# kabachuha/sd-webui-text2video

Measured on NVIDIA H100. Metric: denoised frames/sec (UNet+VAE) ModelScope 24fx256^2 50-step, higher is better.
Workload: dtype f16 (fp32 accumulate / norms / softmax)

## Files before the change

sd-webui-text2video_b200/csrc/api.cu:

```cuda
#include "../../include/t2v_b200.h"
#include "common.cuh"
#include "gemm_tc.cuh"
#include "kernels.cuh"

#include <cstdarg>
#include <cstdlib>
#include <cstdio>
#include <cstring>

namespace t2v {

static char g_err[512] = "";
static int g_device = -1;
static int g_num_sms = 132;
static void* g_gn_ws = nullptr;
static size_t g_gn_ws_bytes = 0;

void set_error(const char* fmt, ...) {
    va_list ap;
    va_start(ap, fmt);
    vsnprintf(g_err, sizeof(g_err), fmt, ap);
    va_end(ap);
}
int num_sms() { return g_num_sms; }
// ... 55 lines not shown
}
const char* t2v_last_error(void) { return g_err; }
int t2v_num_sms(void) { return g_num_sms; }
const char* t2v_version(void) { return "t2v_b200 0.2 (sm_90a; wgmma+TMA implicit GEMM)"; }

int t2v_op_gemm(const void* a, long long lda, int K, int nd, const int* dims, int ntaps, const int* tap_off,
                const void* w_packed, int n_alloc, int N, int b_batch_dim, int flags, void* out, long long ldo,
                const void* bias, int bias_rows, long long bias_stride, const void* residual, long long ldr,
                float alpha, int force_bn, int force_cg, void* stream) {
    GemmProblem p;
    memset(&p, 0, sizeof(p));
    p.a = reinterpret_cast<const __half*>(a);
    p.lda = lda;
    p.K = K;
    p.nd = nd;
    for (int d = 0; d < nd; ++d) p.dim[d] = dims[d];
    p.ntaps = ntaps;
    for (int t = 0; t < ntaps; ++t)
        for (int d = 0; d < nd; ++d) p.tap_off[t][d] = tap_off ? tap_off[t * nd + d] : 0;
    p.b = reinterpret_cast<const __half*>(w_packed);
    p.n_alloc = n_alloc;
    p.N = N;
    p.b_batch_dim = b_batch_dim;
    p.flags = flags & ~(GEMM_DBG_FORCE_BS | GEMM_DBG_NO_BS);
    p.force_bs = (flags & GEMM_DBG_FORCE_BS) ? 1 : ((flags & GEMM_DBG_NO_BS) ? -1 : 0);
    p.out = out;
    p.ldo = ldo;
    p.bias = reinterpret_cast<const __half*>(bias);
    p.bias_rows = bias_rows;
    p.bias_stride = bias_stride;
    p.residual = reinterpret_cast<const __half*>(residual);
    p.ldr = ldr;
    p.alpha = alpha;
    p.force_bn = force_bn;
    p.force_cg = force_cg;
    GemmPlan plan;
    int rc = gemm_plan(p, &plan, g_num_sms);
    if (rc != 0) {
        set_error("gemm_plan failed (%d)", rc);
        return rc;
    }
    rc = gemm_launch(plan, reinterpret_cast<cudaStream_t>(stream));
    if (rc != 0) set_error("gemm_launch failed: %s", cudaGetErrorString(cudaGetLastError()));
    return rc;
}

int t2v_latent_blend(const float* image_latents, int image_frames, const double* noise, const double* weights, double* out,
                     double* mask_out, int BC, int F, long long hw, void* stream) {
// ... 116 lines not shown
```

sd-webui-text2video_b200/csrc/gemm_tc.cu:

```cuda
#include "common.cuh"
#include "gemm_tc.cuh"
#include "ptx.cuh"

#include <algorithm>
#include <cstdio>
#include <cstdlib>
#include <cstring>

namespace t2v {

namespace {

constexpr int kThreads = 384;
constexpr int kRegsProducer = 40;
constexpr int kRegsConsumer = 232;
constexpr int kABytes = GEMM_BLOCK_M * GEMM_BLOCK_K * 2;
constexpr int kSmemBudget = 216 * 1024;
constexpr int kMaxStages = 8;
constexpr int kEpiRowBytes = 128;
constexpr int kEpiWarpBytes = 8 * kEpiRowBytes + 16 * 4;
constexpr int kEpiBytes = 8 * kEpiWarpBytes;

template <int BN>
struct Cfg {
    static constexpr int kBBytes = BN * GEMM_BLOCK_K * 2;
    static constexpr int kStageBytes = kABytes + kBBytes;
    static constexpr int kStages = (kSmemBudget / kStageBytes) > kMaxStages ? kMaxStages : (kSmemBudget / kStageBytes);
    static constexpr int kColBytes = BN * 8;
    static constexpr int kTailBytes = 1024  + 256  + kEpiBytes + kColBytes;
    static constexpr int kSmemBytes = kStages * kStageBytes + kTailBytes;
    static constexpr int kBsSmemBytes = kSmemBudget + kTailBytes;
    static_assert(kSmemBytes <= 227 * 1024, "shared memory per block");
};

__device__ __forceinline__ float gelu_erf(float x) {
    const float z = fabsf(x) * 0.70710678118654752440f;
    float t;
    asm("rcp.approx.ftz.f32 %0, %1;" : "=f"(t) : "f"(fmaf(0.3275911f, z, 1.0f)));
    float p = fmaf(t, 0.5f * 1.061405429f, 0.5f * -1.453152027f);
    p = fmaf(p, t, 0.5f * 1.421413741f);
    p = fmaf(p, t, 0.5f * -0.284496736f);
    p = fmaf(p, t, 0.5f * 0.254829592f);
    const float q = p * t * ex2_approx(z * z * -1.4426950408889634f);
    return x * (x < 0.f ? q : 1.0f - q);
}

__device__ __forceinline__ uint32_t stg_off(int r, int b, int segs) {
    const int L = r * segs + (b >> 4);
    return static_cast<uint32_t>(((L ^ ((L >> 3) & 7)) << 4) | (b & 15));
}

template <int BN, bool GEGLU>
__device__ __forceinline__ void epilogue_affine(const GemmDesc& g, float (&acc)[BN / 2], const uint8_t* cols, const int* rowg,
                                                const float2 (&rs)[2], int tn, int lane) {
    const int quad = lane & 3, fr = lane >> 2;
    if (g.bias != nullptr && g.bias_rows > 0 && (g.flags & GEMM_LN) == 0) {
        const int nvalid = GEGLU ? g.N / 2 : g.N;
        const __half* brow[2];
#pragma unroll
        for (int h = 0; h < 2; ++h) {
            const int fg = rowg[fr + 8 * h];
            brow[h] = g.bias + (fg >= 0 ? (fg / g.bias_rows) * g.bias_stride : 0);
        }
#pragma unroll
        for (int j = 0; j < BN / 8; ++j) {
#pragma unroll
            for (int e = 0; e < 2; ++e) {
                const int col = tn * BN + 8 * j + 2 * quad + e;
                if (!GEGLU && col >= nvalid) continue;
                acc[4 * j + e] = fmaf(acc[4 * j + e], g.alpha, __half2float(__ldg(brow[0] + col)));
                acc[4 * j + 2 + e] = fmaf(acc[4 * j + 2 + e], g.alpha, __half2float(__ldg(brow[1] + col)));
            }
        }
        return;
    }
    const bool ln = (g.flags & GEMM_LN) != 0;
#pragma unroll
    for (int j = 0; j < BN / 8; ++j) {
        const int c = 8 * j + 2 * quad;
        if (ln) {
            const float4 p = *reinterpret_cast<const float4*>(cols + 8 * c);
            acc[4 * j] = fmaf(rs[0].y, fmaf(-rs[0].x, p.x, acc[4 * j]), p.y);
            acc[4 * j + 2] = fmaf(rs[1].y, fmaf(-rs[1].x, p.x, acc[4 * j + 2]), p.y);
            acc[4 * j + 1] = fmaf(rs[0].y, fmaf(-rs[0].x, p.z, acc[4 * j + 1]), p.w);
            acc[4 * j + 3] = fmaf(rs[1].y, fmaf(-rs[1].x, p.z, acc[4 * j + 3]), p.w);
        } else {
            const float2 b = __half22float2(*reinterpret_cast<const __half2*>(cols + 2 * c));
            acc[4 * j] = fmaf(acc[4 * j], g.alpha, b.x);
            acc[4 * j + 2] = fmaf(acc[4 * j + 2], g.alpha, b.x);
            acc[4 * j + 1] = fmaf(acc[4 * j + 1], g.alpha, b.y);
            acc[4 * j + 3] = fmaf(acc[4 * j + 3], g.alpha, b.y);
        }
    }
}
// ... 91 lines not shown
            const int idx = lane + 32 * p;
            if (idx >= 8 * segs) continue;
            const int gr = rowg[8 * h + idx / segs];
            if (gr < 0) continue;
            const int col = ocol0 + c * CW + EPS * (idx % segs);
            const uint4 val = *reinterpret_cast<const uint4*>(stg + stg_off(idx / segs, 16 * (idx % segs), segs));
            uint8_t* dst = static_cast<uint8_t*>(g.out) + ((F32 ? sp * g.split_stride : 0) + gr * g.ldo + col) * ES;
            if (vec_out && col + EPS <= nvalid) {
                *reinterpret_cast<uint4*>(dst) = val;
            } else {
                const uint32_t w[4] = {val.x, val.y, val.z, val.w};
#pragma unroll
                for (int e = 0; e < EPS; ++e)
                    if (col + e < nvalid) {
                        if constexpr (F32) reinterpret_cast<uint32_t*>(dst)[e] = w[e];
                        else reinterpret_cast<uint16_t*>(dst)[e] = static_cast<uint16_t>(w[e >> 1] >> (16 * (e & 1)));
                    }
            }
        }
        __syncwarp();
    }
}

template <int BN, bool GEGLU, int CG, bool BS = false>
__global__ void __launch_bounds__(kThreads, 1) gemm_tc_kernel(const __grid_constant__ GemmDesc g) {
    using Cf = Cfg<BN>;
    static_assert(!BS || CG == 1, "B-stationary tiles are single-CTA");
    static_assert(!BS || Cf::kBsSmemBytes <= 227 * 1024, "shared memory per block");
    constexpr int kBarStages = BS ? kMaxStages : Cf::kStages;
    const uint32_t rank = CG == 2 ? cluster_ctarank() : 0u;
    extern __shared__ uint8_t smem_raw[];
    const uint32_t raw = smem_u32(smem_raw);
    uint8_t* smem = smem_raw + (((raw + 1023u) & ~1023u) - raw);
    uint64_t* bars = reinterpret_cast<uint64_t*>(smem + (BS ? kSmemBudget : Cf::kStages * Cf::kStageBytes));
    uint64_t* full = bars;
    uint64_t* empty = bars + kBarStages;
    uint64_t* bfull = empty + kBarStages;
    uint64_t* colfull = bfull + 1;
    uint64_t* colempty = bfull + 2;
    uint8_t* const epi = reinterpret_cast<uint8_t*>(bars) + 256;
    uint8_t* const cols = epi + kEpiBytes;
    const int nst = BS ? g.bs_stages : Cf::kStages;
    uint8_t* const sB_res = smem;
    uint8_t* const sA_ring = smem + (BS ? g.ntaps * g.k_chunks * Cf::kBBytes : 0);

    const int wg = threadIdx.x >> 7;

    if (threadIdx.x == 0) {
        tma_prefetch_desc(&g.map_a);
        tma_prefetch_desc(&g.map_b);
        for (int i = 0; i < kBarStages; ++i) {
            mbar_init(&full[i], 1);
            mbar_init(&empty[i], 2 * CG);
        }
        if constexpr (BS) mbar_init(bfull, 1);
        mbar_init(colfull, 1);
        mbar_init(colempty, 8);
        fence_barrier_init();
    }
    if constexpr (CG == 2) cluster_sync_all();
    else __syncthreads();
    griddep_wait();

    const int pairs_m = (g.tiles_m + CG - 1) / CG;
    const int nsplit = g.splits > 1 ? g.splits : 1;
    const int total_pairs = pairs_m * g.tiles_n * nsplit;
    const int k_total = g.ntaps * g.k_chunks;
    const int k_per = g.splits > 1 ? g.k_per_split : k_total;
    const int bs_tn = BS ? static_cast<int>(blockIdx.x) % g.tiles_n : 0;
    const int first_pair = BS ? static_cast<int>(blockIdx.x) / g.tiles_n : static_cast<int>(blockIdx.x) / CG;
    const int pair_stride = BS ? (static_cast<int>(gridDim.x) - bs_tn + g.tiles_n - 1) / g.tiles_n : static_cast<int>(gridDim.x) / CG;
    const int total_items = BS ? g.tiles_m : total_pairs;
    const bool col_operands = (g.flags & GEMM_LN) != 0 || g.bias == nullptr || g.bias_rows == 0;

    if (wg == 0) {
        setmaxnreg_dec<kRegsProducer>();
        if (threadIdx.x < 32 && elect_one()) {
            int stage = 0;
            uint32_t phase = 0;
            if constexpr (BS) {
// ... 4 lines not shown
                        tma_load_3d(sB_res + it * Cf::kBBytes, &g.map_b, bfull, kc * GEMM_BLOCK_K, bs_tn * BN, tap);
                        if (++kc == kch0) {
                            kc = 0;
                            ++tap;
                        }
                    }
                }
            }
            const int kch = g.k_chunks, nd = g.nd, a_tx = g.a_tx_bytes, tiles_n_ = g.tiles_n, tiles_m_ = g.tiles_m;
            const int bdim = g.b_batch_dim;
            for (int wi = first_pair; wi < total_items; wi += pair_stride) {
                int sp = 0, pt = wi;
                if (!BS && nsplit > 1) {
                    sp = wi % nsplit;
                    pt = wi / nsplit;
                }
                const int it0 = sp * k_per, it1 = min(k_total, it0 + k_per);
                int tn = bs_tn, tmi = wi;
                if constexpr (!BS) {
                    const int pm = pt / tiles_n_;
                    tn = pt - pm * tiles_n_;
                    tmi = pm * CG + static_cast<int>(rank);
                }
                int org[GEMM_MAX_RDIMS] = {0, 0, 0, 0};
                if (nd == 1) {
                    org[0] = tmi * g.box[0];
                } else {
                    int tm = tmi;
#pragma unroll
                    for (int d = 0; d < GEMM_MAX_RDIMS; ++d) {
                        if (d < nd) {
                            const int td = g.tdim[d];
                            const int qd = tm / td;
                            org[d] = (tm - qd * td) * g.box[d];
                            tm = qd;
                        }
                    }
                }
                if (tmi >= tiles_m_) org[0] = g.dim[0];
                const int bbatch = bdim < 0 ? 0 : (bdim == 0 ? org[0] : (bdim == 1 ? org[1] : (bdim == 2 ? org[2] : org[3])));
                int tap = 0, kc = it0;
                if (it0 >= kch) {
                    tap = it0 / kch;
                    kc = it0 - tap * kch;
                }
                int c1 = org[0] + g.tap_off[tap][0], c2 = org[1] + g.tap_off[tap][1];
                int c3 = org[2] + g.tap_off[tap][2], c4 = org[3] + g.tap_off[tap][3];
                for (int it = it0; it < it1; ++it) {
                    mbar_wait(&empty[stage], phase ^ 1u);
                    uint8_t* sa = BS ? sA_ring + stage * kABytes : smem + stage * Cf::kStageBytes;
                    uint8_t* sb = sa + kABytes;
                    const int k0 = kc * GEMM_BLOCK_K;
                    mbar_expect_tx(&full[stage], static_cast<uint32_t>(a_tx + (BS ? 0 : Cf::kBBytes)));
                    if (nd == 1) tma_load_2d(sa, &g.map_a, &full[stage], k0, c1);
                    else if (nd == 2) tma_load_3d(sa, &g.map_a, &full[stage], k0, c1, c2);
                    else if (nd == 3) tma_load_4d(sa, &g.map_a, &full[stage], k0, c1, c2, c3);
                    else tma_load_5d(sa, &g.map_a, &full[stage], k0, c1, c2, c3, c4);
                    if constexpr (CG == 2) {
                        constexpr int kHalf = BN / 2;
                        tma_load_3d_mc(sb + rank * (kHalf * GEMM_BLOCK_K * 2), &g.map_b, &full[stage], k0,
                                       tn * BN + static_cast<int>(rank) * kHalf, tap + bbatch, static_cast<uint16_t>(3));
// ... 18 lines not shown
            }
            griddep_launch();
        } else if (threadIdx.x >= 32 && threadIdx.x < 64 && col_operands) {
            const int lane = threadIdx.x & 31;
            const bool ln = (g.flags & GEMM_LN) != 0;
            uint32_t cphase = 0;
            for (int wi = first_pair; wi < total_items; wi += pair_stride) {
                const int col0 = (BS ? bs_tn : (wi / nsplit) % g.tiles_n) * BN;
                mbar_wait(colempty, cphase ^ 1u);
#pragma unroll
                for (int c = lane; c < BN; c += 32) {
                    const int col = col0 + c;
                    if (ln) {
                        reinterpret_cast<float2*>(cols)[c] =
                            col < g.N ? make_float2(__ldg(g.colsum + col), __ldg(g.bias32 + col)) : make_float2(0.f, 0.f);
                    } else {
                        reinterpret_cast<__half*>(cols)[c] = g.bias != nullptr && col < g.N ? __ldg(g.bias + col) : __ushort_as_half(0);
                    }
                }
                __syncwarp();
                if (lane == 0) mbar_arrive(colfull);
                cphase ^= 1u;
            }
        }
        __syncwarp();
    } else {
        setmaxnreg_inc<kRegsConsumer>();
        const int cw = wg - 1;
        const int lt = threadIdx.x & 127;
        const int wr = lt >> 5, lane = lt & 31;
        int stage = 0;
        uint32_t phase = 0;
        if constexpr (BS) {
            if (first_pair < total_items) mbar_wait(bfull, 0u);
        }
        const bool out_f32 = (g.flags & GEMM_OUT_F32) != 0;
        const bool ln = (g.flags & GEMM_LN) != 0;
        uint8_t* const stg = epi + (cw * 4 + wr) * kEpiWarpBytes;
        int* const rowg = reinterpret_cast<int*>(stg + 8 * kEpiRowBytes);
        uint32_t cphase = 0;
        float acc[BN / 2];
        uint4 rq[ResQ<BN>::kDepth][2];
        for (int wi = first_pair; wi < total_items; wi += pair_stride) {
            const int sp = BS ? 0 : wi % nsplit;
            const int pt = wi / nsplit;
            const int tn = BS ? bs_tn : pt % g.tiles_n;
            const int tmi = BS ? wi : (pt / g.tiles_n) * CG + static_cast<int>(rank);
            const int it0s = BS ? 0 : sp * k_per;
            const int k_iters = min(k_total, it0s + k_per) - it0s;

            if (lane < 16) {
                const int r = cw * 64 + wr * 16 + lane;
                int grow = -1;
                if (tmi < g.tiles_m) {
                    if (g.nd == 1) {
                        const int o = tmi * g.box[0];
                        if (r < g.box[0] && o + r < g.dim[0]) grow = o + r;
                    } else {
                        int tm = tmi, rr = r;
                        long long mul = 1, gr = 0;
                        bool valid = true;
#pragma unroll
                        for (int d = 0; d < GEMM_MAX_RDIMS; ++d) {
                            const int td = g.tdim[d];
                            const int c = (tm % td) * g.box[d] + rr % g.box[d];
                            tm /= td;
                            rr /= g.box[d];
                            valid = valid && (c < g.dim[d]);
                            gr += mul * c;
                            mul *= g.dim[d];
                        }
                        if (valid && rr == 0) grow = static_cast<int>(gr);
// ... 15 lines not shown
            for (int it = 0; it < k_iters; ++it) {
                mbar_wait(&full[stage], phase);
                const uint32_t sa = smem_u32(BS ? sA_ring + stage * kABytes : smem + stage * Cf::kStageBytes) + cw * (64 * 128);
                const uint32_t sb = BS ? smem_u32(sB_res + it * Cf::kBBytes) : smem_u32(smem + stage * Cf::kStageBytes) + kABytes;
                const uint64_t da = wgmma_desc_sw128(sa);
                const uint64_t db = wgmma_desc_sw128(sb);
                wgmma_fence();
#pragma unroll
                for (int k = 0; k < GEMM_BLOCK_K / 16; ++k)
                    wgmma_ss<BN>(acc, da + static_cast<uint64_t>(k * 2), db + static_cast<uint64_t>(k * 2), (it | k) != 0 ? 1u : 0u);
                wgmma_commit();
                wgmma_wait<1>();
                if (prev >= 0 && lt == 0) {
                    mbar_arrive(&empty[prev]);
                    if constexpr (CG == 2) mbar_arrive_cluster(&empty[prev], rank ^ 1u);
                }
                prev = stage;
                if (++stage == nst) {
                    stage = 0;
                    phase ^= 1u;
                }
            }
            if constexpr (!GEGLU) {
                if (g.residual != nullptr) {
#pragma unroll
                    for (int u = 0; u < ResQ<BN>::kDepth; ++u) ResQ<BN>::load(g, rowg, tn, u, lane, rq[u]);
                }
            }
            wgmma_wait<0>();
#pragma unroll
            for (int i = 0; i < BN / 2; ++i) reg_fence(acc[i]);
            if (prev >= 0 && lt == 0) {
                mbar_arrive(&empty[prev]);
                if constexpr (CG == 2) mbar_arrive_cluster(&empty[prev], rank ^ 1u);
            }

            if (col_operands) mbar_wait(colfull, cphase);
            epilogue_affine<BN, GEGLU>(g, acc, cols, rowg, rs, tn, lane);
            if (col_operands) {
                __syncwarp();
                if (lane == 0) mbar_arrive(colempty);
                cphase ^= 1u;
            }
            if constexpr (GEGLU) epilogue_warp<BN, true, false>(g, acc, rq, stg, rowg, tn, sp, lane);
            else if (out_f32) epilogue_warp<BN, false, true>(g, acc, rq, stg, rowg, tn, sp, lane);
            else epilogue_warp<BN, false, false>(g, acc, rq, stg, rowg, tn, sp, lane);
        }
    }
    if constexpr (CG == 2) cluster_sync_all();
}

typedef CUresult (*EncodeTiledFn)(CUtensorMap*, CUtensorMapDataType, cuuint32_t, void*, const cuuint64_t*,
                                  const cuuint64_t*, const cuuint32_t*, const cuuint32_t*, CUtensorMapInterleave,
                                  CUtensorMapSwizzle, CUtensorMapL2promotion, CUtensorMapFloatOOBfill);
EncodeTiledFn g_encode = nullptr;
bool g_inited = false;

int encode_map(CUtensorMap* m, const void* base, int rank, const cuuint64_t* dims, const cuuint64_t* strides_bytes,
               const cuuint32_t* box) {
    cuuint32_t estr[5] = {1, 1, 1, 1, 1};
    CUresult r = g_encode(m, CU_TENSOR_MAP_DATA_TYPE_FLOAT16, static_cast<cuuint32_t>(rank), const_cast<void*>(base),
                          dims, strides_bytes, box, estr, CU_TENSOR_MAP_INTERLEAVE_NONE, CU_TENSOR_MAP_SWIZZLE_128B,
                          CU_TENSOR_MAP_L2_PROMOTION_L2_256B, CU_TENSOR_MAP_FLOAT_OOB_FILL_NONE);
    if (r != CUDA_SUCCESS) {
        fprintf(stderr, "[t2v] cuTensorMapEncodeTiled failed: %d (rank %d, dims %llu %llu %llu %llu %llu)\n",
                static_cast<int>(r), rank, (unsigned long long)dims[0], (unsigned long long)(rank > 1 ? dims[1] : 0),
                (unsigned long long)(rank > 2 ? dims[2] : 0), (unsigned long long)(rank > 3 ? dims[3] : 0),
                (unsigned long long)(rank > 4 ? dims[4] : 0));
        return -1;
    }
    return 0;
}

struct Variant {
    int bn, geglu, cg, smem;
    const void* fn;
    int bs;
};
template <int BN, bool G, int CG>
Variant variant() {
    return Variant{BN, G ? 1 : 0, CG, Cfg<BN>::kSmemBytes, reinterpret_cast<const void*>(&gemm_tc_kernel<BN, G, CG>), 0};
}
template <int BN, bool G>
Variant variant_bs() {
    return Variant{BN, G ? 1 : 0, 1, Cfg<BN>::kBsSmemBytes, reinterpret_cast<const void*>(&gemm_tc_kernel<BN, G, 1, true>), 1};
}
const Variant* variants(int* n) {
    static const Variant v[] = {
        variant<16, false, 1>(),  variant<64, false, 1>(),  variant<128, false, 1>(), variant<160, false, 1>(),
        variant<192, false, 1>(), variant<224, false, 1>(),
        variant<256, false, 1>(), variant<64, true, 1>(),   variant<128, true, 1>(),  variant<256, true, 1>(),
        variant<64, false, 2>(),  variant<128, false, 2>(), variant<160, false, 2>(), variant<256, false, 2>(),
        variant<64, true, 2>(),   variant<128, true, 2>(),  variant<256, true, 2>(),
        variant_bs<160, false>(), variant_bs<128, false>(), variant_bs<128, true>(), variant_bs<64, false>(),
    };
    *n = static_cast<int>(sizeof(v) / sizeof(v[0]));
    return v;
}
const Variant* find_variant(int bn, bool geglu, int cg, int bs = 0) {
    int n;
    const Variant* v = variants(&n);
    for (int i = 0; i < n; ++i)
        if (v[i].bn == bn && v[i].geglu == (geglu ? 1 : 0) && v[i].cg == cg && v[i].bs == bs) return &v[i];
    return nullptr;
}

}

int gemm_init() {
    if (g_inited) return 0;
    void* fn = nullptr;
    cudaDriverEntryPointQueryResult qres;
    if (cudaGetDriverEntryPoint("cuTensorMapEncodeTiled", &fn, cudaEnableDefault, &qres) != cudaSuccess ||
        fn == nullptr) {
        fprintf(stderr, "[t2v] cuTensorMapEncodeTiled entry point not found\n");
        return -1;
    }
    g_encode = reinterpret_cast<EncodeTiledFn>(fn);
    int nv = 0;
    const Variant* vs = variants(&nv);
    bool attr_fail = false;
    for (int i = 0; i < nv; ++i)
        if (cudaFuncSetAttribute(vs[i].fn, cudaFuncAttributeMaxDynamicSharedMemorySize, vs[i].smem) != cudaSuccess) attr_fail = true;
    if (attr_fail) {
        fprintf(stderr, "[t2v] cudaFuncSetAttribute(max dynamic smem) failed: %s\n",
                cudaGetErrorString(cudaGetLastError()));
// ... 188 lines not shown
    {
        cuuint64_t dims[5], strides[4];
        cuuint32_t box[5];
        dims[0] = static_cast<cuuint64_t>(p.K);
        box[0] = GEMM_BLOCK_K;
        long long pitch = p.lda * 2;
        for (int d = 0; d < p.nd; ++d) {
            dims[d + 1] = static_cast<cuuint64_t>(g.dim[d]);
            box[d + 1] = static_cast<cuuint32_t>(g.box[d]);
            strides[d] = static_cast<cuuint64_t>(pitch);
            pitch *= g.dim[d];
        }
        if (encode_map(&g.map_a, p.a, p.nd + 1, dims, strides, box) != 0) return -5;
    }
    {
        const int nb = p.b_batch_dim >= 0 ? g.dim[p.b_batch_dim] : p.ntaps;
        cuuint64_t dims[3] = {static_cast<cuuint64_t>(p.K), static_cast<cuuint64_t>(p.n_alloc),
                              static_cast<cuuint64_t>(nb)};
        const cuuint64_t ldb = static_cast<cuuint64_t>(p.ldb > 0 ? p.ldb : p.K);
        cuuint64_t strides[2] = {ldb * 2, ldb * 2 * static_cast<cuuint64_t>(p.n_alloc)};
        cuuint32_t box[3] = {GEMM_BLOCK_K, static_cast<cuuint32_t>(bn / plan->cg), 1};
        if (encode_map(&g.map_b, p.b, 3, dims, strides, box) != 0) return -6;
    }
    const Variant* var = find_variant(bn, (p.flags & GEMM_GEGLU) != 0, plan->cg, plan->bs);
    if (var == nullptr) return -7;
    const int kt = g.ntaps * g.k_chunks;
    g.k_per_split = (kt + g.splits - 1) / g.splits;
    g.splits = (kt + g.k_per_split - 1) / g.k_per_split;
    const long long pairs = static_cast<long long>((g.tiles_m + plan->cg - 1) / plan->cg) * g.tiles_n * g.splits;
    plan->grid = plan->cg * static_cast<int>(std::min<long long>(pairs, num_sms / plan->cg));
    if (plan->bs) plan->grid = (num_sms / g.tiles_n) * g.tiles_n;
    plan->smem = var->smem;
    plan->flops = 2.0 * static_cast<double>(rows) * p.N * p.K * p.ntaps;
    return 0;
}

int gemm_launch(const GemmPlan& plan, cudaStream_t stream) {
    const Variant* var = find_variant(plan.bn, (plan.desc.flags & GEMM_GEGLU) != 0, plan.cg, plan.bs);
    if (var == nullptr) return -1;
    cudaLaunchConfig_t cfg;
    memset(&cfg, 0, sizeof(cfg));
    cfg.gridDim = dim3(static_cast<unsigned>(plan.grid));
    cfg.blockDim = dim3(static_cast<unsigned>(kThreads));
    cfg.dynamicSmemBytes = static_cast<size_t>(plan.smem);
    cfg.stream = stream;
    cudaLaunchAttribute attr[2];
    unsigned na = 0;
    if (plan.cg == 2) {
        attr[na].id = cudaLaunchAttributeClusterDimension;
        attr[na].val.clusterDim.x = 2;
        attr[na].val.clusterDim.y = 1;
        attr[na].val.clusterDim.z = 1;
        ++na;
    }
    if (pdl_enabled()) {
        attr[na].id = cudaLaunchAttributeProgrammaticStreamSerialization;
        attr[na].val.programmaticStreamSerializationAllowed = 1;
        ++na;
    }
    cfg.attrs = attr;
    cfg.numAttrs = na;
// ... 6 lines not shown
```

sd-webui-text2video_b200/csrc/gemm_tc.cuh:

```cuda
#pragma once
#include <cuda.h>
#include <cuda_fp16.h>
#include <cuda_runtime.h>
#include <stdint.h>

namespace t2v {

constexpr int GEMM_BLOCK_M = 128;
constexpr int GEMM_BLOCK_K = 64;
constexpr int GEMM_MAX_TAPS = 9;
constexpr int GEMM_MAX_RDIMS = 4;

enum GemmFlags : int {
    GEMM_GEGLU = 1,
    GEMM_OUT_F32 = 2,
    GEMM_LN = 4,
    GEMM_DBG_FORCE_BS = 2048,
    GEMM_DBG_NO_BS = 4096,
};

struct GemmDesc {
    CUtensorMap map_a;
    CUtensorMap map_b;
    int nd;
    int dim[GEMM_MAX_RDIMS];
    int box[GEMM_MAX_RDIMS];
    int tdim[GEMM_MAX_RDIMS];
    int tiles_m, tiles_n;
    int ntaps, k_chunks;
    int8_t tap_off[GEMM_MAX_TAPS][GEMM_MAX_RDIMS];
    int b_batch_dim;
    int a_tx_bytes;
    int N;
    int flags;
    void* out;
    long long ldo;
    const __half* bias;
    int bias_rows;
    long long bias_stride;
    const __half* residual;
    long long ldr;
    float alpha;
    const float2* rowstat;
    const float* colsum;
    const float* bias32;
    int splits;
// ... 12 lines not shown
    int tap_off[GEMM_MAX_TAPS][GEMM_MAX_RDIMS];
    const __half* b;
    long long ldb;
    int n_alloc;
    int N;
    int b_batch_dim;
    int flags;
    void* out;
    long long ldo;
    const __half* bias;
    int bias_rows;
    long long bias_stride;
    const __half* residual;
    long long ldr;
    float alpha;
    int force_bn;
    int force_cg;
    const float2* rowstat;
    const float* colsum;
    const float* bias32;
    int splits;
    long long split_stride;
    int force_bs;
};

struct GemmPlan {
    GemmDesc desc;
    int bn;
    int cg;
    int bs;
    int grid;
    int smem;
    double flops;
};

int gemm_bs_bn(long long tiles_m, int N, int K, int ntaps, bool geglu, int num_sms, int force_bn = 0, bool any_k = false,
               int* stages_out = nullptr);
int gemm_plan(const GemmProblem& p, GemmPlan* plan, int num_sms);
int gemm_launch(const GemmPlan& plan, cudaStream_t stream);
int gemm_init();
int tma_encode_f16(CUtensorMap* m, const void* base, int rank, const unsigned long long* dims,
                   const unsigned long long* strides_bytes, const unsigned* box);

}
```

sd-webui-text2video_b200/csrc/ptx.cuh:

```cuda
#pragma once
#include <cuda_fp16.h>
#include <cuda_runtime.h>
#include <stdint.h>

namespace t2v {

__device__ __forceinline__ uint32_t smem_u32(const void* p) {
    return static_cast<uint32_t>(__cvta_generic_to_shared(p));
}

__device__ __forceinline__ bool elect_one() {
    uint32_t pred = 0;
    asm volatile(
        "{\n\t.reg .b32 rx;\n\t.reg .pred px;\n\t"
        "elect.sync rx|px, 0xffffffff;\n\t"
        "selp.b32 %0, 1, 0, px;\n\t}"
        : "=r"(pred));
    return pred != 0;
}

__device__ __forceinline__ void mbar_init(uint64_t* bar, uint32_t count) {
    asm volatile("mbarrier.init.shared::cta.b64 [%0], %1;" ::"r"(smem_u32(bar)), "r"(count));
}
__device__ __forceinline__ void fence_barrier_init() {
    asm volatile("fence.mbarrier_init.release.cluster;" ::: "memory");
}
__device__ __forceinline__ void mbar_expect_tx(uint64_t* bar, uint32_t bytes) {
    asm volatile("mbarrier.arrive.expect_tx.shared::cta.b64 _, [%0], %1;" ::"r"(smem_u32(bar)), "r"(bytes)
                 : "memory");
}
__device__ __forceinline__ void mbar_arrive(uint64_t* bar) {
    asm volatile("mbarrier.arrive.shared::cta.b64 _, [%0];" ::"r"(smem_u32(bar)) : "memory");
}
__device__ __forceinline__ void mbar_arrive_cluster(uint64_t* bar, uint32_t cta) {
    asm volatile(
        "{\n\t.reg .b32 ra;\n\t"
        "mapa.shared::cluster.u32 ra, %0, %1;\n\t"
        "mbarrier.arrive.release.cluster.shared::cluster.b64 _, [ra];\n\t}"
        ::"r"(smem_u32(bar)), "r"(cta)
        : "memory");
}
// ... 45 lines not shown
        "[%2];" ::"r"(smem_u32(dst)),
        "l"(map), "r"(smem_u32(bar)), "r"(c0), "r"(c1), "r"(c2), "r"(c3)
        : "memory");
}
__device__ __forceinline__ void tma_load_5d(void* dst, const void* map, uint64_t* bar, int c0, int c1, int c2,
                                            int c3, int c4) {
    asm volatile(
        "cp.async.bulk.tensor.5d.shared::cluster.global.mbarrier::complete_tx::bytes [%0], [%1, {%3, %4, %5, %6, "
        "%7}], [%2];" ::"r"(smem_u32(dst)),
        "l"(map), "r"(smem_u32(bar)), "r"(c0), "r"(c1), "r"(c2), "r"(c3), "r"(c4)
        : "memory");
}
__device__ __forceinline__ void tma_load_3d_mc(void* dst, const void* map, uint64_t* bar, int c0, int c1, int c2,
                                               uint16_t mask) {
    asm volatile(
        "cp.async.bulk.tensor.3d.shared::cluster.global.mbarrier::complete_tx::bytes.multicast::cluster [%0], [%1, {%3, %4, "
        "%5}], [%2], %6;" ::"r"(smem_u32(dst)),
        "l"(map), "r"(smem_u32(bar)), "r"(c0), "r"(c1), "r"(c2), "h"(mask)
        : "memory");
}
__device__ __forceinline__ void tma_prefetch_desc(const void* map) {
    asm volatile("prefetch.tensormap [%0];" ::"l"(map) : "memory");
}

__device__ __forceinline__ uint64_t wgmma_desc_sw128(uint32_t smem_addr) {
    uint64_t d = 0;
    d |= static_cast<uint64_t>((smem_addr & 0x3FFFF) >> 4);
    d |= static_cast<uint64_t>(1) << 16;
    d |= static_cast<uint64_t>(1024 >> 4) << 32;
    d |= static_cast<uint64_t>(1) << 62;
    return d;
}
__device__ __forceinline__ void wgmma_fence() { asm volatile("wgmma.fence.sync.aligned;" ::: "memory"); }
__device__ __forceinline__ void wgmma_commit() { asm volatile("wgmma.commit_group.sync.aligned;" ::: "memory"); }
template <int N>
__device__ __forceinline__ void wgmma_wait() {
    asm volatile("wgmma.wait_group.sync.aligned %0;" ::"n"(N) : "memory");
}
__device__ __forceinline__ void reg_fence(float& r) { asm volatile("" : "+f"(r)::"memory"); }
template <int N>
__device__ __forceinline__ void wgmma_ss(float* d, uint64_t da, uint64_t db, uint32_t scale_d);
template <>
__device__ __forceinline__ void wgmma_ss<16>(float* d, uint64_t da, uint64_t db, uint32_t scale_d) {
    asm volatile(
        "{\n\t.reg .pred p;\n\tsetp.ne.b32 p, %10, 0;\n\t"
        "wgmma.mma_async.sync.aligned.m64n16k16.f32.f16.f16 "
// ... 122 lines not shown
```

sd-webui-text2video_b200/t2v_b200/ops.py:

```python
import ctypes as C

import torch

from . import _lib

GEMM_GEGLU = 1
GEMM_FORCE_BS, GEMM_NO_BS = 2048, 4096
GEMM_OUT_F32 = 2


def _ia(vals):
    return (C.c_int * len(vals))(*[int(v) for v in vals])


def gemm(a, w_packed, N, *, K=None, lda=None, dims=None, taps=None, n_alloc=None, b_batch_dim=-1, flags=0, out=None,
         ldo=None, bias=None, bias_rows=0, bias_stride=0, residual=None, ldr=None, alpha=1.0, force_bn=0, force_cg=0):
    l = _lib.lib()
    rows = a.shape[0]
    K = K if K is not None else a.shape[1]
    lda = lda if lda is not None else a.stride(0)
    dims = list(dims) if dims is not None else [rows]
    nd = len(dims)
    taps = taps if taps is not None else [[0] * nd]
    flat = [o for t in taps for o in t]
    n_alloc = n_alloc if n_alloc is not None else w_packed.shape[-2]
    ncols = N // 2 if (flags & GEMM_GEGLU) else N
    if out is None:
        out = torch.empty((rows, ncols), device=a.device, dtype=torch.float32 if (flags & GEMM_OUT_F32) else torch.float16)
    ldo = ldo if ldo is not None else out.stride(0)
    ldr = ldr if ldr is not None else (residual.stride(0) if residual is not None else 0)
    rc = l.t2v_op_gemm(_lib.ptr(a), lda, K, nd, _ia(dims), len(taps), _ia(flat), _lib.ptr(w_packed), n_alloc, N,
# ... 90 lines not shown
```

Before: 12.33.

## Stage full output tile in shared memory and write it with TMA stores

Adds a TMA-store epilogue. Consumer warps write the whole output tile into swizzled shared memory, and a dedicated warp loads the residual tile with TMA beforehand and stores the finished tile with bulk tensor stores. The goal is to replace per-warp strided global stores and register-staged residual loads with coalesced asynchronous bulk transfers that overlap the next tile's mainloop. The output tile takes shared memory away from the pipeline ring, which lowers stage counts for wide tiles. A slab fallback variant keeps deeper rings for BN 224/256 when the grid has at most one tile per SM.

```diff
diff --git a/sd-webui-text2video_b200/csrc/api.cu b/sd-webui-text2video_b200/csrc/api.cu
--- a/sd-webui-text2video_b200/csrc/api.cu
+++ b/sd-webui-text2video_b200/csrc/api.cu
@@ -101,8 +101,9 @@
     p.n_alloc = n_alloc;
     p.N = N;
     p.b_batch_dim = b_batch_dim;
-    p.flags = flags & ~(GEMM_DBG_FORCE_BS | GEMM_DBG_NO_BS);
+    p.flags = flags & ~(GEMM_DBG_FORCE_BS | GEMM_DBG_NO_BS | GEMM_DBG_SLAB_OUT);
     p.force_bs = (flags & GEMM_DBG_FORCE_BS) ? 1 : ((flags & GEMM_DBG_NO_BS) ? -1 : 0);
+    p.slab_out = (flags & GEMM_DBG_SLAB_OUT) ? 1 : 0;
     p.out = out;
     p.ldo = ldo;
     p.bias = reinterpret_cast<const __half*>(bias);
diff --git a/sd-webui-text2video_b200/csrc/gemm_tc.cu b/sd-webui-text2video_b200/csrc/gemm_tc.cu
--- a/sd-webui-text2video_b200/csrc/gemm_tc.cu
+++ b/sd-webui-text2video_b200/csrc/gemm_tc.cu
@@ -15,23 +15,32 @@
 constexpr int kRegsProducer = 40;
 constexpr int kRegsConsumer = 232;
 constexpr int kABytes = GEMM_BLOCK_M * GEMM_BLOCK_K * 2;
+constexpr int kSmemPerBlock = 227 * 1024;
 constexpr int kSmemBudget = 216 * 1024;
 constexpr int kMaxStages = 8;
 constexpr int kEpiRowBytes = 128;
-constexpr int kEpiWarpBytes = 8 * kEpiRowBytes + 16 * 4;
-constexpr int kEpiBytes = 8 * kEpiWarpBytes;
-
-template <int BN>
+constexpr int kSlabBytes = 8 * 8 * kEpiRowBytes;
+constexpr int kRowTabBytes = 8 * 16 * 4;
+
+__host__ __device__ constexpr int out_chunk_cols(int outw) { return outw >= 32 ? 32 : 16; }
+__host__ __device__ constexpr int out_chunks(int outw) { return (outw + out_chunk_cols(outw) - 1) / out_chunk_cols(outw); }
+
+template <int BN, bool SLAB = false>
 struct Cfg {
     static constexpr int kBBytes = BN * GEMM_BLOCK_K * 2;
     static constexpr int kStageBytes = kABytes + kBBytes;
-    static constexpr int kStages = (kSmemBudget / kStageBytes) > kMaxStages ? kMaxStages : (kSmemBudget / kStageBytes);
     static constexpr int kColBytes = BN * 8;
-    static constexpr int kTailBytes = 1024  + 256  + kEpiBytes + kColBytes;
-    static constexpr int kSmemBytes = kStages * kStageBytes + kTailBytes;
-    static constexpr int kBsSmemBytes = kSmemBudget + kTailBytes;
-    static_assert(kSmemBytes <= 227 * 1024, "shared memory per block");
+    static constexpr int kTailBytes = 1024  + 256  + kRowTabBytes + kColBytes;
+    static constexpr int kOutBytes = SLAB ? kSlabBytes : std::max(kSlabBytes, out_chunks(BN) * GEMM_BLOCK_M * out_chunk_cols(BN) * 2);
+    static constexpr int kStages = std::min(kMaxStages, (kSmemPerBlock - kTailBytes - kOutBytes) / kStageBytes);
+    static constexpr int kSmemBytes = kStages * kStageBytes + kOutBytes + kTailBytes;
+    static constexpr int kBsSmemBytes = kSmemBudget + kSlabBytes + kTailBytes;
+    static_assert(kSmemBytes <= kSmemPerBlock, "shared memory per block");
 };
+static_assert(Cfg<256>::kStages == 3 && Cfg<224>::kStages == 3 && Cfg<192>::kStages == 4 && Cfg<160>::kStages == 5 &&
+                  Cfg<128>::kStages == 6 && Cfg<64>::kStages == 8 && Cfg<16>::kStages == 8,
+              "ring depths next to the output tile");
+static_assert(Cfg<256, true>::kStages == 4 && Cfg<224, true>::kStages == 4, "ring depths without the output tile");
 
 __device__ __forceinline__ float gelu_erf(float x) {
     const float z = fabsf(x) * 0.70710678118654752440f;
@@ -54,22 +63,22 @@
 __device__ __forceinline__ void epilogue_affine(const GemmDesc& g, float (&acc)[BN / 2], const uint8_t* cols, const int* rowg,
                                                 const float2 (&rs)[2], int tn, int lane) {
     const int quad = lane & 3, fr = lane >> 2;
-    if (g.bias != nullptr && g.bias_rows > 0 && (g.flags & GEMM_LN) == 0) {
-        const int nvalid = GEGLU ? g.N / 2 : g.N;
+    if (!GEGLU && g.bias != nullptr && g.bias_rows > 0 && (g.flags & GEMM_LN) == 0) {
+        const int col0 = tn * BN + 2 * quad;
+        const int nrem = g.N - col0;
         const __half* brow[2];
 #pragma unroll
         for (int h = 0; h < 2; ++h) {
             const int fg = rowg[fr + 8 * h];
-            brow[h] = g.bias + (fg >= 0 ? (fg / g.bias_rows) * g.bias_stride : 0);
+            brow[h] = g.bias + (fg >= 0 ? (fg / g.bias_rows) * g.bias_stride : 0) + col0;
         }
 #pragma unroll
         for (int j = 0; j < BN / 8; ++j) {
 #pragma unroll
             for (int e = 0; e < 2; ++e) {
-                const int col = tn * BN + 8 * j + 2 * quad + e;
-                if (!GEGLU && col >= nvalid) continue;
-                acc[4 * j + e] = fmaf(acc[4 * j + e], g.alpha, __half2float(__ldg(brow[0] + col)));
-                acc[4 * j + 2 + e] = fmaf(acc[4 * j + 2 + e], g.alpha, __half2float(__ldg(brow[1] + col)));
+                if (8 * j + e >= nrem) continue;
+                acc[4 * j + e] = fmaf(acc[4 * j + e], g.alpha, __half2float(__ldg(brow[0] + 8 * j + e)));
+                acc[4 * j + 2 + e] = fmaf(acc[4 * j + 2 + e], g.alpha, __half2float(__ldg(brow[1] + 8 * j + e)));
             }
         }
         return;
@@ -207,24 +216,109 @@
     }
 }
 
-template <int BN, bool GEGLU, int CG, bool BS = false>
+__device__ __forceinline__ void tile_origin(const GemmDesc& g, int tmi, int (&org)[GEMM_MAX_RDIMS]) {
+#pragma unroll
+    for (int d = 0; d < GEMM_MAX_RDIMS; ++d) org[d] = 0;
+    if (g.nd == 1) {
+        org[0] = tmi * g.box[0];
+        return;
+    }
+    int tm = tmi;
+#pragma unroll
+    for (int d = 0; d < GEMM_MAX_RDIMS; ++d) {
+        if (d < g.nd) {
+            const int td = g.tdim[d];
+            const int qd = tm / td;
+            org[d] = (tm - qd * td) * g.box[d];
+            tm = qd;
+        }
+    }
+}
+
+__device__ __forceinline__ void tma_store_box(const CUtensorMap* map, const void* src, int nd, int c0, const int (&org)[GEMM_MAX_RDIMS]) {
+    if (nd == 1) tma_store_2d(map, src, c0, org[0]);
+    else if (nd == 2) tma_store_3d(map, src, c0, org[0], org[1]);
+    else if (nd == 3) tma_store_4d(map, src, c0, org[0], org[1], org[2]);
+    else tma_store_5d(map, src, c0, org[0], org[1], org[2], org[3]);
+}
+__device__ __forceinline__ void tma_load_box(void* dst, const CUtensorMap* map, uint64_t* bar, int nd, int c0,
+                                             const int (&org)[GEMM_MAX_RDIMS]) {
+    if (nd == 1) tma_load_2d(dst, map, bar, c0, org[0]);
+    else if (nd == 2) tma_load_3d(dst, map, bar, c0, org[0], org[1]);
+    else if (nd == 3) tma_load_4d(dst, map, bar, c0, org[0], org[1], org[2]);
+    else tma_load_5d(dst, map, bar, c0, org[0], org[1], org[2], org[3]);
+}
+
+template <int OCW>
+__device__ __forceinline__ int out_unit_swizzle(int r) { return ((r * OCW * 2) >> 7) & (OCW / 8 - 1); }
+
+template <int BN, bool GEGLU>
+__device__ __forceinline__ int live_out_chunks(const GemmDesc& g, int tn) {
+    constexpr int OUTW = GEGLU ? BN / 2 : BN;
+    constexpr int OCW = out_chunk_cols(OUTW);
+    return min(out_chunks(OUTW), ((GEGLU ? g.N / 2 : g.N) - tn * OUTW + OCW - 1) / OCW);
+}
+
+template <int BN, bool GEGLU>
+__device__ __forceinline__ void epilogue_tile(const GemmDesc& g, const float (&acc)[BN / 2], uint8_t* tile, uint64_t* tilefree,
+                                              uint32_t tphase, uint64_t* tilefull, int r0, int lane) {
+    constexpr int OUTW = GEGLU ? BN / 2 : BN;
+    constexpr int OCW = out_chunk_cols(OUTW);
+    const int quad = lane & 3, fr = lane >> 2;
+    const bool has_res = !GEGLU && g.residual != nullptr;
+    const uint32_t row = smem_u32(tile) + static_cast<uint32_t>((r0 + fr) * (OCW * 2) + 4 * quad);
+    const int sw = out_unit_swizzle<OCW>(r0 + fr);
+    mbar_wait(tilefree, tphase);
+#pragma unroll
+    for (int j = 0; j < OUTW / 8; ++j) {
+#pragma unroll
+        for (int h = 0; h < 2; ++h) {
+            const uint32_t p = row + (j / (OCW / 8)) * (GEMM_BLOCK_M * OCW * 2) + 8 * h * (OCW * 2) + (((j % (OCW / 8)) ^ sw) << 4);
+            float v0 = acc[4 * j + 2 * h], v1 = acc[4 * j + 2 * h + 1];
+            __half2 v;
+            if constexpr (GEGLU) {
+                const __half2 xh = __floats2half2_rn(v0, v1);
+                const float2 gf = __half22float2(__floats2half2_rn(acc[BN / 4 + 4 * j + 2 * h], acc[BN / 4 + 4 * j + 2 * h + 1]));
+                v = __hmul2(xh, __floats2half2_rn(gelu_erf(gf.x), gelu_erf(gf.y)));
+            } else {
+                if (has_res) {
+                    const uint32_t rw = ld_shared_u32(p);
+                    const float2 f = __half22float2(*reinterpret_cast<const __half2*>(&rw));
+                    v0 += f.x;
+                    v1 += f.y;
+                }
+                v = __floats2half2_rn(v0, v1);
+            }
+            st_shared_u32(p, *reinterpret_cast<const uint32_t*>(&v));
+        }
+    }
+    fence_proxy_async_smem();
+    __syncwarp();
+    if (lane == 0) mbar_arrive(tilefull);
+}
+
+template <int BN, bool GEGLU, int CG, bool BS = false, bool SLAB = false>
 __global__ void __launch_bounds__(kThreads, 1) gemm_tc_kernel(const __grid_constant__ GemmDesc g) {
-    using Cf = Cfg<BN>;
+    using Cf = Cfg<BN, SLAB>;
     static_assert(!BS || CG == 1, "B-stationary tiles are single-CTA");
-    static_assert(!BS || Cf::kBsSmemBytes <= 227 * 1024, "shared memory per block");
+    static_assert(!BS || Cf::kBsSmemBytes <= kSmemPerBlock, "shared memory per block");
     constexpr int kBarStages = BS ? kMaxStages : Cf::kStages;
     const uint32_t rank = CG == 2 ? cluster_ctarank() : 0u;
     extern __shared__ uint8_t smem_raw[];
     const uint32_t raw = smem_u32(smem_raw);
     uint8_t* smem = smem_raw + (((raw + 1023u) & ~1023u) - raw);
-    uint64_t* bars = reinterpret_cast<uint64_t*>(smem + (BS ? kSmemBudget : Cf::kStages * Cf::kStageBytes));
+    uint8_t* const epi = smem + (BS ? kSmemBudget : Cf::kStages * Cf::kStageBytes);
+    uint64_t* bars = reinterpret_cast<uint64_t*>(epi + (BS ? kSlabBytes : Cf::kOutBytes));
     uint64_t* full = bars;
     uint64_t* empty = bars + kBarStages;
     uint64_t* bfull = empty + kBarStages;
     uint64_t* colfull = bfull + 1;
     uint64_t* colempty = bfull + 2;
-    uint8_t* const epi = reinterpret_cast<uint8_t*>(bars) + 256;
-    uint8_t* const cols = epi + kEpiBytes;
+    uint64_t* tilefree = bfull + 3;
+    uint64_t* tilefull = bfull + 4;
+    int* const rowtab = reinterpret_cast<int*>(reinterpret_cast<uint8_t*>(bars) + 256);
+    uint8_t* const cols = reinterpret_cast<uint8_t*>(rowtab) + kRowTabBytes;
+    const bool tma_out = !BS && !SLAB && g.tma_out != 0;
     const int nst = BS ? g.bs_stages : Cf::kStages;
     uint8_t* const sB_res = smem;
     uint8_t* const sA_ring = smem + (BS ? g.ntaps * g.k_chunks * Cf::kBBytes : 0);
@@ -234,6 +328,10 @@
     if (threadIdx.x == 0) {
         tma_prefetch_desc(&g.map_a);
         tma_prefetch_desc(&g.map_b);
+        if (tma_out) {
+            tma_prefetch_desc(&g.map_o);
+            if (g.residual != nullptr) tma_prefetch_desc(&g.map_r);
+        }
         for (int i = 0; i < kBarStages; ++i) {
             mbar_init(&full[i], 1);
             mbar_init(&empty[i], 2 * CG);
@@ -241,6 +339,8 @@
         if constexpr (BS) mbar_init(bfull, 1);
         mbar_init(colfull, 1);
         mbar_init(colempty, 8);
+        mbar_init(tilefree, 1);
+        mbar_init(tilefull, 8);
         fence_barrier_init();
     }
     if constexpr (CG == 2) cluster_sync_all();
@@ -291,21 +391,8 @@
                     tn = pt - pm * tiles_n_;
                     tmi = pm * CG + static_cast<int>(rank);
                 }
-                int org[GEMM_MAX_RDIMS] = {0, 0, 0, 0};
-                if (nd == 1) {
-                    org[0] = tmi * g.box[0];
-                } else {
-                    int tm = tmi;
-#pragma unroll
-                    for (int d = 0; d < GEMM_MAX_RDIMS; ++d) {
-                        if (d < nd) {
-                            const int td = g.tdim[d];
-                            const int qd = tm / td;
-                            org[d] = (tm - qd * td) * g.box[d];
-                            tm = qd;
-                        }
-                    }
-                }
+                int org[GEMM_MAX_RDIMS];
+                tile_origin(g, tmi, org);
                 if (tmi >= tiles_m_) org[0] = g.dim[0];
                 const int bbatch = bdim < 0 ? 0 : (bdim == 0 ? org[0] : (bdim == 1 ? org[1] : (bdim == 2 ? org[2] : org[3])));
                 int tap = 0, kc = it0;
@@ -370,6 +457,36 @@
                 if (lane == 0) mbar_arrive(colfull);
                 cphase ^= 1u;
             }
+        } else if (threadIdx.x >= 64 && threadIdx.x < 96 && tma_out) {
+            if (elect_one()) {
+                constexpr int OUTW = GEGLU ? BN / 2 : BN;
+                constexpr int OCW = out_chunk_cols(OUTW);
+                constexpr int kChunkBytes = GEMM_BLOCK_M * OCW * 2;
+                const bool has_res = !GEGLU && g.residual != nullptr;
+                const uint32_t box_bytes = static_cast<uint32_t>(g.a_tx_bytes / GEMM_BLOCK_K * OCW);
+                uint32_t fphase = 0;
+                for (int wi = first_pair; wi < total_items; wi += pair_stride) {
+                    const int pt = wi / nsplit;
+                    const int tn = pt % g.tiles_n;
+                    const int tmi = (pt / g.tiles_n) * CG + static_cast<int>(rank);
+                    const int nch = tmi < g.tiles_m ? live_out_chunks<BN, GEGLU>(g, tn) : 0;
+                    int org[GEMM_MAX_RDIMS];
+                    tile_origin(g, tmi, org);
+                    if (has_res && nch > 0) {
+                        mbar_expect_tx(tilefree, nch * box_bytes);
+                        for (int c = 0; c < nch; ++c)
+                            tma_load_box(epi + c * kChunkBytes, &g.map_r, tilefree, g.nd, tn * OUTW + c * OCW, org);
+                    } else {
+                        mbar_arrive(tilefree);
+                    }
+                    mbar_wait(tilefull, fphase);
+                    fphase ^= 1u;
+                    for (int c = 0; c < nch; ++c) tma_store_box(&g.map_o, epi + c * kChunkBytes, g.nd, tn * OUTW + c * OCW, org);
+                    bulk_commit_group();
+                    bulk_wait_group_read_0();
+                }
+                bulk_wait_group_0();
+            }
         }
         __syncwarp();
     } else {
@@ -384,9 +501,9 @@
         }
         const bool out_f32 = (g.flags & GEMM_OUT_F32) != 0;
         const bool ln = (g.flags & GEMM_LN) != 0;
-        uint8_t* const stg = epi + (cw * 4 + wr) * kEpiWarpBytes;
-        int* const rowg = reinterpret_cast<int*>(stg + 8 * kEpiRowBytes);
-        uint32_t cphase = 0;
+        uint8_t* const stg = epi + (cw * 4 + wr) * (8 * kEpiRowBytes);
+        int* const rowg = rowtab + (cw * 4 + wr) * 16;
+        uint32_t cphase = 0, tphase = 0;
         float acc[BN / 2];
         uint4 rq[ResQ<BN>::kDepth][2];
         for (int wi = first_pair; wi < total_items; wi += pair_stride) {
@@ -395,7 +512,7 @@
             const int tn = BS ? bs_tn : pt % g.tiles_n;
             const int tmi = BS ? wi : (pt / g.tiles_n) * CG + static_cast<int>(rank);
             const int it0s = BS ? 0 : sp * k_per;
-            const int k_iters = min(k_total, it0s + k_per) - it0s;
+            const int k_iters = min(g.ntaps * g.k_chunks, it0s + k_per) - it0s;
 
             if (lane < 16) {
                 const int r = cw * 64 + wr * 16 + lane;
@@ -457,7 +574,7 @@
                 }
             }
             if constexpr (!GEGLU) {
-                if (g.residual != nullptr) {
+                if (!tma_out && g.residual != nullptr) {
 #pragma unroll
                     for (int u = 0; u < ResQ<BN>::kDepth; ++u) ResQ<BN>::load(g, rowg, tn, u, lane, rq[u]);
                 }
@@ -470,6 +587,8 @@
                 if constexpr (CG == 2) mbar_arrive_cluster(&empty[prev], rank ^ 1u);
             }
 
+            uint32_t ring = static_cast<uint32_t>(stage) | (phase << 16);
+            asm volatile("" : "+r"(ring));
             if (col_operands) mbar_wait(colfull, cphase);
             epilogue_affine<BN, GEGLU>(g, acc, cols, rowg, rs, tn, lane);
             if (col_operands) {
@@ -477,9 +596,19 @@
                 if (lane == 0) mbar_arrive(colempty);
                 cphase ^= 1u;
             }
-            if constexpr (GEGLU) epilogue_warp<BN, true, false>(g, acc, rq, stg, rowg, tn, sp, lane);
-            else if (out_f32) epilogue_warp<BN, false, true>(g, acc, rq, stg, rowg, tn, sp, lane);
-            else epilogue_warp<BN, false, false>(g, acc, rq, stg, rowg, tn, sp, lane);
+            if (tma_out) {
+                epilogue_tile<BN, GEGLU>(g, acc, epi, tilefree, tphase, tilefull, cw * 64 + wr * 16, lane);
+                tphase ^= 1u;
+            } else if constexpr (GEGLU) {
+                epilogue_warp<BN, true, false>(g, acc, rq, stg, rowg, tn, sp, lane);
+            } else if (out_f32) {
+                epilogue_warp<BN, false, true>(g, acc, rq, stg, rowg, tn, sp, lane);
+            } else {
+                epilogue_warp<BN, false, false>(g, acc, rq, stg, rowg, tn, sp, lane);
+            }
+            asm volatile("" : "+r"(ring));
+            stage = static_cast<int>(ring & 0xffffu);
+            phase = ring >> 16;
         }
     }
     if constexpr (CG == 2) cluster_sync_all();
@@ -492,10 +621,10 @@
 bool g_inited = false;
 
 int encode_map(CUtensorMap* m, const void* base, int rank, const cuuint64_t* dims, const cuuint64_t* strides_bytes,
-               const cuuint32_t* box) {
+               const cuuint32_t* box, CUtensorMapSwizzle swizzle = CU_TENSOR_MAP_SWIZZLE_128B) {
     cuuint32_t estr[5] = {1, 1, 1, 1, 1};
     CUresult r = g_encode(m, CU_TENSOR_MAP_DATA_TYPE_FLOAT16, static_cast<cuuint32_t>(rank), const_cast<void*>(base),
-                          dims, strides_bytes, box, estr, CU_TENSOR_MAP_INTERLEAVE_NONE, CU_TENSOR_MAP_SWIZZLE_128B,
+                          dims, strides_bytes, box, estr, CU_TENSOR_MAP_INTERLEAVE_NONE, swizzle,
                           CU_TENSOR_MAP_L2_PROMOTION_L2_256B, CU_TENSOR_MAP_FLOAT_OOB_FILL_NONE);
     if (r != CUDA_SUCCESS) {
         fprintf(stderr, "[t2v] cuTensorMapEncodeTiled failed: %d (rank %d, dims %llu %llu %llu %llu %llu)\n",
@@ -510,15 +639,19 @@
 struct Variant {
     int bn, geglu, cg, smem;
     const void* fn;
-    int bs;
+    int bs, slab;
 };
 template <int BN, bool G, int CG>
 Variant variant() {
-    return Variant{BN, G ? 1 : 0, CG, Cfg<BN>::kSmemBytes, reinterpret_cast<const void*>(&gemm_tc_kernel<BN, G, CG>), 0};
+    return Variant{BN, G ? 1 : 0, CG, Cfg<BN>::kSmemBytes, reinterpret_cast<const void*>(&gemm_tc_kernel<BN, G, CG>), 0, 0};
 }
 template <int BN, bool G>
 Variant variant_bs() {
-    return Variant{BN, G ? 1 : 0, 1, Cfg<BN>::kBsSmemBytes, reinterpret_cast<const void*>(&gemm_tc_kernel<BN, G, 1, true>), 1};
+    return Variant{BN, G ? 1 : 0, 1, Cfg<BN>::kBsSmemBytes, reinterpret_cast<const void*>(&gemm_tc_kernel<BN, G, 1, true>), 1, 0};
+}
+template <int BN>
+Variant variant_slab() {
+    return Variant{BN, 0, 1, Cfg<BN, true>::kSmemBytes, reinterpret_cast<const void*>(&gemm_tc_kernel<BN, false, 1, false, true>), 0, 1};
 }
 const Variant* variants(int* n) {
     static const Variant v[] = {
@@ -528,15 +661,16 @@
         variant<64, false, 2>(),  variant<128, false, 2>(), variant<160, false, 2>(), variant<256, false, 2>(),
         variant<64, true, 2>(),   variant<128, true, 2>(),  variant<256, true, 2>(),
         variant_bs<160, false>(), variant_bs<128, false>(), variant_bs<128, true>(), variant_bs<64, false>(),
+        variant_slab<224>(),      variant_slab<256>(),
     };
     *n = static_cast<int>(sizeof(v) / sizeof(v[0]));
     return v;
 }
-const Variant* find_variant(int bn, bool geglu, int cg, int bs = 0) {
+const Variant* find_variant(int bn, bool geglu, int cg, int bs, int slab) {
     int n;
     const Variant* v = variants(&n);
     for (int i = 0; i < n; ++i)
-        if (v[i].bn == bn && v[i].geglu == (geglu ? 1 : 0) && v[i].cg == cg && v[i].bs == bs) return &v[i];
+        if (v[i].bn == bn && v[i].geglu == (geglu ? 1 : 0) && v[i].cg == cg && v[i].bs == bs && v[i].slab == slab) return &v[i];
     return nullptr;
 }
 
@@ -771,11 +905,41 @@
         cuuint32_t box[3] = {GEMM_BLOCK_K, static_cast<cuuint32_t>(bn / plan->cg), 1};
         if (encode_map(&g.map_b, p.b, 3, dims, strides, box) != 0) return -6;
     }
-    const Variant* var = find_variant(bn, (p.flags & GEMM_GEGLU) != 0, plan->cg, plan->bs);
-    if (var == nullptr) return -7;
+    const auto tma_rows = [](const void* ptr, long long ld) { return (reinterpret_cast<uintptr_t>(ptr) & 15) == 0 && (ld & 7) == 0; };
+    g.tma_out = !(p.flags & GEMM_OUT_F32) && !plan->bs && !p.slab_out && tma_rows(p.out, p.ldo) &&
+                (p.residual == nullptr || tma_rows(p.residual, p.ldr));
     const int kt = g.ntaps * g.k_chunks;
     g.k_per_split = (kt + g.splits - 1) / g.splits;
     g.splits = (kt + g.k_per_split - 1) / g.k_per_split;
+    const long long tiles_all = static_cast<long long>(g.tiles_m) * g.tiles_n * g.splits;
+    plan->slab = !plan->bs && plan->cg == 1 && !(p.flags & GEMM_GEGLU) && (bn == 224 || bn == 256) &&
+                 (!g.tma_out || tiles_all <= num_sms) ? 1 : 0;
+    if (plan->slab) g.tma_out = 0;
+    if (g.tma_out) {
+        const int outw = (p.flags & GEMM_GEGLU) ? bn / 2 : bn;
+        const int ocw = out_chunk_cols(outw);
+        cuuint64_t dims[5];
+        cuuint64_t strides[4];
+        cuuint32_t box[5];
+        dims[0] = static_cast<cuuint64_t>((p.flags & GEMM_GEGLU) ? p.N / 2 : p.N);
+        box[0] = static_cast<cuuint32_t>(ocw);
+        for (int d = 0; d < p.nd; ++d) {
+            dims[d + 1] = static_cast<cuuint64_t>(g.dim[d]);
+            box[d + 1] = static_cast<cuuint32_t>(g.box[d]);
+        }
+        const CUtensorMapSwizzle sw = ocw == 32 ? CU_TENSOR_MAP_SWIZZLE_64B : CU_TENSOR_MAP_SWIZZLE_32B;
+        for (int which = 0; which < (p.residual != nullptr ? 2 : 1); ++which) {
+            long long pitch = (which == 0 ? p.ldo : p.ldr) * 2;
+            for (int d = 0; d < p.nd; ++d) {
+                strides[d] = static_cast<cuuint64_t>(pitch);
+                pitch *= g.dim[d];
+            }
+            if (encode_map(which == 0 ? &g.map_o : &g.map_r, which == 0 ? p.out : p.residual, p.nd + 1, dims, strides, box, sw) != 0)
+                return -8;
+        }
+    }
+    const Variant* var = find_variant(bn, (p.flags & GEMM_GEGLU) != 0, plan->cg, plan->bs, plan->slab);
+    if (var == nullptr) return -7;
     const long long pairs = static_cast<long long>((g.tiles_m + plan->cg - 1) / plan->cg) * g.tiles_n * g.splits;
     plan->grid = plan->cg * static_cast<int>(std::min<long long>(pairs, num_sms / plan->cg));
     if (plan->bs) plan->grid = (num_sms / g.tiles_n) * g.tiles_n;
@@ -785,7 +949,7 @@
 }
 
 int gemm_launch(const GemmPlan& plan, cudaStream_t stream) {
-    const Variant* var = find_variant(plan.bn, (plan.desc.flags & GEMM_GEGLU) != 0, plan.cg, plan.bs);
+    const Variant* var = find_variant(plan.bn, (plan.desc.flags & GEMM_GEGLU) != 0, plan.cg, plan.bs, plan.slab);
     if (var == nullptr) return -1;
     cudaLaunchConfig_t cfg;
     memset(&cfg, 0, sizeof(cfg));
diff --git a/sd-webui-text2video_b200/csrc/gemm_tc.cuh b/sd-webui-text2video_b200/csrc/gemm_tc.cuh
--- a/sd-webui-text2video_b200/csrc/gemm_tc.cuh
+++ b/sd-webui-text2video_b200/csrc/gemm_tc.cuh
@@ -17,11 +17,15 @@
     GEMM_LN = 4,
     GEMM_DBG_FORCE_BS = 2048,
     GEMM_DBG_NO_BS = 4096,
+    GEMM_DBG_SLAB_OUT = 8192,
 };
 
 struct GemmDesc {
     CUtensorMap map_a;
     CUtensorMap map_b;
+    CUtensorMap map_o;
+    CUtensorMap map_r;
+    int tma_out;
     int nd;
     int dim[GEMM_MAX_RDIMS];
     int box[GEMM_MAX_RDIMS];
@@ -80,6 +84,7 @@
     int splits;
     long long split_stride;
     int force_bs;
+    int slab_out;
 };
 
 struct GemmPlan {
@@ -87,6 +92,7 @@
     int bn;
     int cg;
     int bs;
+    int slab;
     int grid;
     int smem;
     double flops;
diff --git a/sd-webui-text2video_b200/csrc/ptx.cuh b/sd-webui-text2video_b200/csrc/ptx.cuh
--- a/sd-webui-text2video_b200/csrc/ptx.cuh
+++ b/sd-webui-text2video_b200/csrc/ptx.cuh
@@ -17,6 +17,15 @@
         "selp.b32 %0, 1, 0, px;\n\t}"
         : "=r"(pred));
     return pred != 0;
+}
+
+__device__ __forceinline__ uint32_t ld_shared_u32(uint32_t addr) {
+    uint32_t v;
+    asm volatile("ld.shared.u32 %0, [%1];" : "=r"(v) : "r"(addr) : "memory");
+    return v;
+}
+__device__ __forceinline__ void st_shared_u32(uint32_t addr, uint32_t v) {
+    asm volatile("st.shared.u32 [%0], %1;" ::"r"(addr), "r"(v) : "memory");
 }
 
 __device__ __forceinline__ void mbar_init(uint64_t* bar, uint32_t count) {
@@ -108,6 +117,31 @@
 __device__ __forceinline__ void tma_prefetch_desc(const void* map) {
     asm volatile("prefetch.tensormap [%0];" ::"l"(map) : "memory");
 }
+
+__device__ __forceinline__ void tma_store_2d(const void* map, const void* src, int c0, int c1) {
+    asm volatile("cp.async.bulk.tensor.2d.global.shared::cta.bulk_group [%0, {%2, %3}], [%1];"
+                 ::"l"(map), "r"(smem_u32(src)), "r"(c0), "r"(c1)
+                 : "memory");
+}
+__device__ __forceinline__ void tma_store_3d(const void* map, const void* src, int c0, int c1, int c2) {
+    asm volatile("cp.async.bulk.tensor.3d.global.shared::cta.bulk_group [%0, {%2, %3, %4}], [%1];"
+                 ::"l"(map), "r"(smem_u32(src)), "r"(c0), "r"(c1), "r"(c2)
+                 : "memory");
+}
+__device__ __forceinline__ void tma_store_4d(const void* map, const void* src, int c0, int c1, int c2, int c3) {
+    asm volatile("cp.async.bulk.tensor.4d.global.shared::cta.bulk_group [%0, {%2, %3, %4, %5}], [%1];"
+                 ::"l"(map), "r"(smem_u32(src)), "r"(c0), "r"(c1), "r"(c2), "r"(c3)
+                 : "memory");
+}
+__device__ __forceinline__ void tma_store_5d(const void* map, const void* src, int c0, int c1, int c2, int c3, int c4) {
+    asm volatile("cp.async.bulk.tensor.5d.global.shared::cta.bulk_group [%0, {%2, %3, %4, %5, %6}], [%1];"
+                 ::"l"(map), "r"(smem_u32(src)), "r"(c0), "r"(c1), "r"(c2), "r"(c3), "r"(c4)
+                 : "memory");
+}
+__device__ __forceinline__ void bulk_commit_group() { asm volatile("cp.async.bulk.commit_group;" ::: "memory"); }
+__device__ __forceinline__ void bulk_wait_group_read_0() { asm volatile("cp.async.bulk.wait_group.read 0;" ::: "memory"); }
+__device__ __forceinline__ void bulk_wait_group_0() { asm volatile("cp.async.bulk.wait_group 0;" ::: "memory"); }
+__device__ __forceinline__ void fence_proxy_async_smem() { asm volatile("fence.proxy.async.shared::cta;" ::: "memory"); }
 
 __device__ __forceinline__ uint64_t wgmma_desc_sw128(uint32_t smem_addr) {
     uint64_t d = 0;
diff --git a/sd-webui-text2video_b200/t2v_b200/ops.py b/sd-webui-text2video_b200/t2v_b200/ops.py
--- a/sd-webui-text2video_b200/t2v_b200/ops.py
+++ b/sd-webui-text2video_b200/t2v_b200/ops.py
@@ -7,6 +7,7 @@
 GEMM_GEGLU = 1
 GEMM_FORCE_BS, GEMM_NO_BS = 2048, 4096
 GEMM_OUT_F32 = 2
+GEMM_SLAB_OUT = 8192
 
 
 def _ia(vals):
```

After: 12.72 (median of 6 runs). 1.03x the previous value.
